# fjall-rs/lsm-tree

Measured on AMD Instinct MI355X. Metric: device-resident data-block decode+encode GiB/s, 1 M × 4 KiB blocks, higher is better.
Workload: dtype u8; 1 GPU; BASELINE configs[1]/[2]: encode + decode round trip of 1 M x 4 KiB data blocks, device-resident; blocks_per_gpu=1048576, items_per_gpu=54525952, block_bytes_per_gpu=3953267212, restart_interval=16, key_len=16, val_len=64, parallelism=shard1 (independent block batches, no collective)

## Files before the change

### lsm-tree_amd/csrc/encode.hip

```cpp
#include <hip/hip_runtime.h>

#include <math.h>

#include <algorithm>
#include <cstddef>
#include <type_traits>

#include "block_format.hpp"
#include "decode.hpp"
#include "encode.hpp"
#include "scan.hpp"
#include "fill.hpp"

namespace lsmgpu {

constexpr uint32_t kPlanHuge = 1, kPlanBad = 2, kPlanMedium = 4, kPlanBig = 8;
constexpr uint32_t kPlanHugeGpu = 16;
constexpr uint32_t kImgMedium = 20 * 1024;
constexpr uint32_t kImgBig = 96 * 1024;
constexpr uint32_t kListBigWaves = 8;
constexpr uint32_t kE3HashChunk = 4096;
constexpr uint64_t kListedOne = 1ULL << 40, kOffMask = kListedOne - 1;

struct alignas(16) BlockPlan {
// ... 285 lines not shown
__device__ __forceinline__ ItemMeta load_item(const EncodeParams& P, uint64_t i, bool& bad) {
  ItemMeta m;
  m.ko = koff<kOW>(P, i);
  const uint64_t kl = koff<kOW>(P, i + 1) - m.ko;
  if (kl > 0xFFFF) bad = true;
  m.klen = (uint32_t)min(kl, (uint64_t)0xFFFF);
  m.seq = gload(P.it.seqno, i);
  m.sh = 0;
  m.e = 0;
  if (is_index(P)) {
    m.vo = gload(P.it.handle_off, i);
    m.vl = gload(P.it.handle_size, i);
    m.vt = 0;
  } else {
    m.vo = voff<kOW>(P, i);
    const uint64_t vl = voff<kOW>(P, i + 1) - m.vo;
    m.vt = gload(P.it.vtype, i);
    if (!valid_vtype(m.vt)) bad = true;
    if (!is_tombstone(m.vt) && vl > 0xFFFFFFFFULL) bad = true;
    m.vl = (uint32_t)vl;
  }
  return m;
}

template <int kOW = 0>
__device__ __forceinline__ ItemMeta load_item_lcp(const EncodeParams& P, uint32_t s, uint32_t j, uint32_t ri,
                                                  bool& bad) {
  const uint64_t i = (uint64_t)s + j;
  ItemMeta m = load_item<kOW>(P, i, bad);
  if (!is_index(P) && j % ri != 0) {
    const uint64_t h = (uint64_t)s + (j / ri) * ri;
    const uint64_t hko = koff<kOW>(P, h);
    const uint32_t hkl = (uint32_t)min(koff<kOW>(P, h + 1) - hko, (uint64_t)0xFFFF);
    m.sh = lcp_global(P.it.keys, hko, m.ko, min(hkl, m.klen));
  }
  return m;
}

__device__ __forceinline__ uint32_t head_len(const EncodeParams& P, const ItemMeta& m, bool head) {
  if (is_index(P)) return 1 + leb_len(m.vo) + leb_len(m.vl) + leb_len(m.seq) + leb_len(m.klen);
  return 1 + leb_len(m.seq) + (head ? leb_len(m.klen) : leb_len(m.sh) + leb_len(m.klen - m.sh));
}

__device__ __forceinline__ uint64_t item_record_len(const EncodeParams& P, const ItemMeta& m, bool head) {
  uint64_t rec = head_len(P, m, head) + m.klen - (head ? 0 : m.sh);
  if (!is_index(P) && !is_tombstone(m.vt)) rec += leb_len(m.vl) + (uint64_t)m.vl;
  return rec;
}

template <class D>
__device__ __forceinline__ uint32_t put_leb(D* dst, uint32_t pos, uint64_t v) {
  while (v >= 0x80) {
    dst[pos++] = (uint8_t)(v | 0x80);
    v >>= 7;
  }
  dst[pos++] = (uint8_t)v;
  return pos;
}

struct RecordCopy {
  SpanCopy<2> key;
  SpanCopy<5> val;
  uint32_t dpos;
  __device__ __forceinline__ void issue(const EncodeParams& P, const ItemMeta& m, bool head, uint32_t dpos_) {
    dpos = dpos_;
    const uint32_t kfrom = head ? 0 : m.sh;
    const uint32_t kpos = dpos_ + head_len(P, m, head);
    key.load(P.it.keys + m.ko + kfrom, m.klen - kfrom, kpos);
    const bool has_val = !is_index(P) && !is_tombstone(m.vt);
    const uint32_t vpos = kpos + m.klen - kfrom + leb_len(m.vl);
    val.load(P.it.vals + (has_val ? m.vo : 0), has_val ? m.vl : 0, vpos);
  }
  template <class D>
  __device__ __forceinline__ void store(const EncodeParams& P, const ItemMeta& m, bool head, D* dst) const {
    uint32_t pos = dpos;
    if (is_index(P)) {
      dst[pos++] = 0;
      pos = put_leb(dst, pos, m.vo);
      pos = put_leb(dst, pos, m.vl);
      pos = put_leb(dst, pos, m.seq);
      put_leb(dst, pos, m.klen);
    } else {
      dst[pos++] = (uint8_t)m.vt;
      pos = put_leb(dst, pos, m.seq);
      if (head) {
        put_leb(dst, pos, m.klen);
      } else {
        pos = put_leb(dst, pos, m.sh);
        put_leb(dst, pos, m.klen - m.sh);
      }
      if (!is_tombstone(m.vt)) put_leb(dst, key.d + key.n, m.vl);
    }
    key.store(dst);
    val.store(dst);
  }
};

template <class D>
__device__ __forceinline__ void store_le(D* dst, uint32_t pos, uint64_t v, uint32_t n) {
  for (uint32_t k = 0; k < n; ++k) dst[pos + k] = (uint8_t)(v >> (8 * k));
}

__device__ __forceinline__ uint32_t key_bucket(const EncodeParams& P, uint64_t ko, uint32_t klen, uint32_t buckets) {
  const uint64_t ka = (uint64_t)(uintptr_t)P.it.keys + ko;
  const uint8_t* kb = reinterpret_cast<const uint8_t*>(ka & ~15ULL);
  const uint32_t kq = (uint32_t)(ka & 15);
  const uint64_t h = xxh3_64_any(klen, BaseReader8{kb, kq}, BaseReader64{kb, kq});
  return (uint32_t)(h % buckets);
}

__device__ __forceinline__ uint32_t bucket_byte(uint32_t lo, uint32_t hi) {
  return lo == 0xFFFFFFFFu ? kHashFree : (lo == hi ? lo : kHashConflict);
}

__device__ __forceinline__ void write_trailer_bytes(uint8_t* dst, uint32_t tp, uint32_t ri, uint32_t step,
                                                    uint32_t bin_len, uint32_t bin_off, uint32_t hash_w,
                                                    uint32_t hash_off, uint32_t items) {
  const int lane = threadIdx.x & 63;
  if (lane >= (int)kTrailerLen) return;
  uint32_t v;
  const int k = lane;
  if (k == 0) v = ri;
  else if (k == 1) v = step;
  else if (k < 6) v = bin_len >> (8 * (k - 2));
  else if (k < 10) v = bin_off >> (8 * (k - 6));
  else if (k < 14) v = hash_w >> (8 * (k - 10));
  else if (k < 18) v = hash_off >> (8 * (k - 14));
  else if (k == 18) v = 1;
  else if (k < 27) v = 0;
  else v = items >> (8 * (k - 27));
  dst[tp + k] = (uint8_t)v;
}

__device__ __forceinline__ void write_header_bytes(uint8_t* dst, uint32_t hp, uint32_t type, uint64_t ck_lo,
                                                   uint64_t ck_hi, uint32_t plen) {
  uint64_t w0 = 0x034D534CULL | ((uint64_t)type << 32) | (ck_lo << 40);
  uint64_t w1 = (ck_lo >> 24) | (ck_hi << 40);
  uint64_t w2 = (ck_hi >> 24) | ((uint64_t)plen << 40);
  uint64_t w3 = ((uint64_t)plen >> 24) | ((uint64_t)plen << 8);
  auto r64 = [&](uint32_t o) -> uint64_t {
    const uint32_t q = o >> 3, sft = (o & 7) * 8;
    const uint64_t a = q == 0 ? w0 : q == 1 ? w1 : q == 2 ? w2 : w3;
    const uint64_t b = q == 0 ? w1 : q == 1 ? w2 : q == 2 ? w3 : 0;
    return sft ? (a >> sft) | (b << (64 - sft)) : a;
  };
  auto r8 = [&](uint32_t o) -> uint32_t { return (uint32_t)(r64(o) & 0xFF); };
  uint64_t hlo, hhi;
  xxh3_128_short(29, r8, r64, hlo, hhi);
  const int lane = threadIdx.x & 63;
  if (lane < 29) dst[hp + lane] = (uint8_t)r8(lane);
  else if (lane < 33) dst[hp + lane] = (uint8_t)((uint32_t)hlo >> (8 * (lane - 29)));
}

__device__ __forceinline__ void write_header_quad(uint8_t* dst, uint32_t hp, uint32_t type, uint64_t ck_lo,
                                                  uint64_t ck_hi, uint32_t plen, int q) {
  const uint64_t w0 = 0x034D534CULL | ((uint64_t)type << 32) | (ck_lo << 40);
  const uint64_t w1 = (ck_lo >> 24) | (ck_hi << 40);
  const uint64_t w2 = (ck_hi >> 24) | ((uint64_t)plen << 40);
  const uint64_t w3 = ((uint64_t)plen >> 24) | ((uint64_t)plen << 8);
  auto r64 = [&](uint32_t o) -> uint64_t {
    const uint32_t qq = o >> 3, sft = (o & 7) * 8;
    const uint64_t a = qq == 0 ? w0 : qq == 1 ? w1 : qq == 2 ? w2 : w3;
    const uint64_t b = qq == 0 ? w1 : qq == 1 ? w2 : qq == 2 ? w3 : 0;
    return sft ? (a >> sft) | (b << (64 - sft)) : a;
  };
  auto r8 = [&](uint32_t o) -> uint32_t { return (uint32_t)(r64(o) & 0xFF); };
  uint64_t hlo, hhi;
  xxh3_128_short(29, r8, r64, hlo, hhi);
  const uint64_t w = q == 0 ? w0 : q == 1 ? w1 : q == 2 ? w2 : (w3 & 0xFFFFFFFFFFULL) | (hlo << 40);
  const uint32_t at = hp + 8 * q;
#pragma unroll
  for (uint32_t i = 0; i < 8; ++i) dst[at + i] = (uint8_t)(w >> (8 * i));
  if (q == 0) dst[hp + 32] = (uint8_t)(hlo >> 24);
}

__device__ __forceinline__ void wave_lds_sync() {
  __builtin_amdgcn_fence(__ATOMIC_RELEASE, "wavefront", "local");
  __builtin_amdgcn_wave_barrier();
  __builtin_amdgcn_fence(__ATOMIC_ACQUIRE, "wavefront", "local");
}

__device__ __forceinline__ void finish_block_lds(const EncodeParams& P, uint32_t b, const BlockPlan& pl, uint32_t n,
                                                 uint32_t ri, uint8_t* img, const uint32_t* hlo, const uint32_t* hhi,
                                                 uint32_t pad, uint32_t total, uint8_t* gdst) {
  const int lane = threadIdx.x & 63;
  const uint32_t step = pl.step_flags & 0xFF;
  const uint32_t plen = total - kHdrLen, p0 = pad + kHdrLen, bin_off = pl.recs + 1;
  if (lane == 0) img[p0 + pl.recs] = kTrailerMarker;
  const uint32_t hash_off = pl.hash_w ? bin_off + pl.bin_len * step : 0;
  for (uint32_t k = lane; k < pl.hash_w; k += kWave) img[p0 + hash_off + k] = (uint8_t)bucket_byte(hlo[k], hhi[k]);
  write_trailer_bytes(img, p0 + plen - kTrailerLen, ri, step, pl.bin_len, bin_off, pl.hash_w, hash_off, n);
  wave_lds_sync();
  if (!(kDiagBuild && (P.diag & 2))) {
    uint64_t ck_lo, ck_hi;
    xxh3_128_wave(img, p0, plen, &kLongSecret, ck_lo, ck_hi);
    write_header_bytes(img, pad, P.type, ck_lo, ck_hi, plen);
  }
  wave_lds_sync();
  const uint32_t chunks = (kDiagBuild && (P.diag & 4)) ? 0 : (pad + total + 15) >> 4;
  for (uint32_t c = lane; c < chunks; c += kWave) {
    const uint32_t lo = c * 16, hi = lo + 16;
    if (lo >= pad && hi <= pad + total) {
      copy_store16(reinterpret_cast<u32x4*>(gdst) + c, reinterpret_cast<const u32x4*>(img)[c]);
    } else {
      for (uint32_t k = max(lo, pad); k < min(hi, pad + total); ++k) gdst[k] = img[k];
    }
  }
  if (lane == 0) P.status[b] = ST_OK;
}

template <int kOW>
__device__ __forceinline__ void write_block_lds(const EncodeParams& P, uint32_t b, uint8_t* smem) {
  const int lane = threadIdx.x & 63;
  const uint32_t s = P.starts[b], e = P.starts[b + 1];
  const uint64_t dst_off = P.block_off[b], dst_end = P.block_off[b + 1];
  const BlockPlan pl = P.plans[b];
  const uint32_t step = pl.step_flags & 0xFF;
  if (dst_end > P.out_cap) {
    if (lane == 0) P.status[b] = ST_OVERFLOW;
    return;
  }
  const uint32_t n = e - s;
  const uint32_t ri = is_index(P) ? 1 : P.ri;
  const uint32_t total = (uint32_t)(dst_end - dst_off);
  const uint64_t dabs = (uint64_t)(uintptr_t)P.out + dst_off;
  const uint32_t pad = (uint32_t)(dabs & 15);
  uint8_t* img = smem;
  uint32_t* hlo = reinterpret_cast<uint32_t*>(smem + ((pad + total + 15) & ~15u) + 32);
  uint32_t* hhi = hlo + ((pl.hash_w + 3) & ~3u);
  for (uint32_t k = lane; k < pl.hash_w; k += kWave) {
    hlo[k] = 0xFFFFFFFFu;
    hhi[k] = 0;
  }
  wave_lds_sync();
  const uint32_t p0 = pad + kHdrLen;
  const uint32_t bin_off = pl.recs + 1;
  uint32_t carry = 0;
  for (uint32_t c = 0; c < n; c += kWave) {
    const uint32_t j = c + lane;
    const bool head = j % ri == 0;
    ItemMeta m;
    RecordCopy rc;
    uint32_t rec = 0;
    if (j < n) {
      bool bad = false;
      m = load_item_lcp<kOW>(P, s, j, ri, bad);
      rec = (uint32_t)item_record_len(P, m, head);
    }
    const uint32_t incl = wave_incl_scan_u32(rec);
    const uint32_t roff = carry + incl - rec;
    if (j < n) {
      rc.issue(P, m, head, p0 + roff);
      rc.store(P, m, head, img);
      if (head) store_le(img, p0 + bin_off + (j / ri) * step, roff, step);
      if (pl.hash_w) {
        const uint32_t bk = key_bucket(P, m.ko, m.klen, pl.hash_w);
        atomicMin(&hlo[bk], j / ri);
        atomicMax(&hhi[bk], j / ri);
      }
    }
    carry += wave_bcast_u32(incl, 63);
  }
  wave_lds_sync();
  finish_block_lds(P, b, pl, n, ri, img, hlo, hhi, pad, total, reinterpret_cast<uint8_t*>(dabs & ~15ULL));
}

template <uint32_t kLW, int kOW>
__device__ __forceinline__ void write_block_lds_mw(const EncodeParams& P, uint32_t b, uint8_t* smem, uint32_t* psum,
                                                   uint64_t* contrib) {
  constexpr uint32_t kT = kLW * kWave;
  const uint32_t tid = threadIdx.x, lane = tid & (kWave - 1);
  const uint32_t wave = __builtin_amdgcn_readfirstlane(tid / kWave);
  const uint32_t s = P.starts[b], e = P.starts[b + 1];
  const uint64_t dst_off = P.block_off[b], dst_end = P.block_off[b + 1];
  const BlockPlan pl = P.plans[b];
  const uint32_t step = pl.step_flags & 0xFF;
  if (dst_end > P.out_cap) {
    if (tid == 0) P.status[b] = ST_OVERFLOW;
    return;
  }
  const uint32_t n = e - s;
  const uint32_t ri = is_index(P) ? 1 : P.ri;
  const uint32_t total = (uint32_t)(dst_end - dst_off);
  const uint64_t dabs = (uint64_t)(uintptr_t)P.out + dst_off;
  const uint32_t pad = (uint32_t)(dabs & 15);
  uint8_t* img = smem;
  uint32_t* hlo = reinterpret_cast<uint32_t*>(smem + ((pad + total + 15) & ~15u) + 32);
  uint32_t* hhi = hlo + ((pl.hash_w + 3) & ~3u);
  for (uint32_t k = tid; k < pl.hash_w; k += kT) {
    hlo[k] = 0xFFFFFFFFu;
    hhi[k] = 0;
  }
  __syncthreads();
  const uint32_t p0 = pad + kHdrLen;
  const uint32_t bin_off = pl.recs + 1;
  uint32_t carry = 0;
  for (uint32_t c = 0; c < n; c += kT) {
    const uint32_t j = c + tid;
    const bool head = j % ri == 0;
    ItemMeta m;
    RecordCopy rc;
    uint32_t rec = 0;
    if (j < n) {
      bool bad = false;
      m = load_item_lcp<kOW>(P, s, j, ri, bad);
      rec = (uint32_t)item_record_len(P, m, head);
    }
// ... 421 lines not shown
          else
            hb = kNeedHash, P.hb_fix[0] = 1;
        }
        P.hbucket[(uint64_t)base + t0 + q] = (uint16_t)hb;
      }
    }
    wave_lds_sync();
    uint32_t nq[kPW];
    uint64_t hq[kPW];
#pragma unroll
    for (uint32_t q = 0; q < kPW; ++q) {
      nq[q] = 0;
      hq[q] = 0;
      wa[q] = wb[q];
      if (ok[q] && jjq[q] % ri != 0) {
        const uint32_t h = base + t0 + q - jjq[q] % ri;
        const bool in = h >= base;
        const uint64_t hko = in ? (uint64_t)wkos[h - base] : hk_ko;
        const uint32_t hkl = in ? wkls[h - base] : hk_kl;
        nq[q] = min(hkl, m[q].klen);
        hq[q] = hko;
        wa[q] = in ? wkwin[h - base] : hk_win;
      }
    }
#pragma unroll
    for (uint32_t q = 0; q < kPW; ++q) {
      if (!nq[q]) continue;
      const uint64_t x0 = wa[q].lo ^ wb[q].lo, x1 = wa[q].hi ^ wb[q].hi;
      const uint32_t n = nq[q];
      uint32_t sh;
      if (x0) sh = min(n, (uint32_t)(__builtin_ctzll(x0) >> 3));
      else if (x1) sh = min(n, 8 + (uint32_t)(__builtin_ctzll(x1) >> 3));
      else sh = n <= 16 ? n : lcp_tail(P.it.keys, hq[q], m[q].ko, n);
      m[q].sh = sh;
    }
    uint64_t rec[kPW], tsum = 0;
#pragma unroll
    for (uint32_t q = 0; q < kPW; ++q) {
      rec[q] = ok[q] ? item_record_len(P, m[q], jjq[q] % ri == 0) : 0;
      tsum += rec[q];
    }
    const uint64_t incl = wave_incl_scan_u64(tsum);
    uint64_t ex = carry + incl - tsum;
    uint64_t exq[kPW];
#pragma unroll
    for (uint32_t q = 0; q < kPW; ++q) {
      exq[q] = ex;
      if (ok[q]) {
        const uint32_t jb = jq[q], jj = jjq[q], ridx = jj / ri;
        const uint32_t n = bst[jb + 1] - bst[jb];
        if (jj == 0) bfirst[jb] = ex;
        if (jj + 1 == n) bend[jb] = ex + rec[q];
        if (jj == ridx * ri && ridx == (n - 1) / ri) lhead[jb] = ex;
      }
      ex += rec[q];
    }
    wave_lds_sync();
#pragma unroll
    for (uint32_t q = 0; q < kPW; ++q) {
      if (ok[q]) {
        const uint32_t jj = jjq[q], ridx = jj / ri;
        const bool head = jj == ridx * ri;
        const uint64_t roff = exq[q] - bfirst[jq[q]];
        const uint32_t x = head ? ridx : m[q].sh;
        P.erec[(uint64_t)base + t0 + q] =
            bst[jq[q] + 1] - bst[jq[q]] > kGItems
                ? (uint32_t)min(roff, (uint64_t)0xFFFFFFFFu)
                : (uint32_t)min(roff, (uint64_t)0x7FFF) | (head ? kErecHead : 0u) | (min(x, 0xFFFFu) << 16);
      }
    }
    carry += wave_bcast_u64(incl, kWave - 1);
    {
      const uint32_t last = min(ie, base + kPWStep) - 1, ll = (last - base) / kPW, lq = (last - base) % kPW;
      uint32_t jsel = jjq[0];
#pragma unroll
      for (uint32_t q = 1; q < kPW; ++q) jsel = lq == q ? jjq[q] : jsel;
      const uint32_t jjl = __builtin_amdgcn_readlane((int)jsel, (int)ll);
      const uint32_t h = last - jjl % ri;
      if (h >= base) {
        hk_ko = wkos[h - base];
        hk_kl = wkls[h - base];
        hk_win = wkwin[h - base];
      }
    }
    wave_lds_sync();
  }
  __syncthreads();
  if (tid >= nb) return;
  const uint32_t b = b0 + tid, s = bst[tid], e = bst[tid + 1];
  bool bad = !mono || e <= s || badf[tid] || start_past_items(P, b + 1);
  const uint32_t n = bad ? 0 : e - s;
  const uint64_t recs = bad ? 0 : bend[tid] - bfirst[tid], last_head = bad ? 0 : lhead[tid] - bfirst[tid];
  const uint32_t bin_len = n ? (n + ri - 1) / ri : 0;
  const uint32_t step = last_head <= 0xFFFF ? 2 : 4;
  const uint32_t buckets = bucket_count(n, P.ratio);
  const uint32_t hash_w = (buckets > 0 && bin_len <= kHashMaxPointers) ? buckets : 0;
  const uint64_t total = kHdrLen + recs + 1 + (uint64_t)bin_len * step + hash_w + kTrailerLen;
  if (recs > 0xFFFFFFF0ULL || total > 0xFFFFFF00ULL) bad = true;
  const uint64_t ks = koff<kOW>(P, s), ke = koff<kOW>(P, e);
  const uint64_t vs = voff<kOW>(P, s), ve = voff<kOW>(P, e);
  uint32_t flags = 0;
  if (bad) {
    flags = kPlanBad;
    P.status[b] = ST_BAD_ARG;
  } else if (!group_fits(n, ke - ks, ve - vs, total, hash_w)) {
    const uint64_t need = e2_need(total, hash_w);
    flags = need <= kImgMedium ? kPlanMedium : need <= kImgBig ? kPlanBig : kPlanHuge;
  }
  const BlockPlan pl{(uint32_t)recs, bin_len, hash_w, step | (flags << 8)};
  const uint64_t size = (bad ? 0 : total) | ((flags & (kPlanMedium | kPlanBig | kPlanHuge)) ? kListedOne : 0);
  P.plans[b] = pl;
  if (kFused) {
    fplan[tid] = pl;
    fsize[tid] = size;
    if (size & ~kOffMask) P.status[b] = ST_INCOMPLETE;
  } else {
    P.sizes[b] = size;
  }
  P.kspan[b] = ks;
  P.vspan[b] = vs;
  if (b + 1 == P.n_blocks) {
    P.kspan[b + 1] = ke;
    P.vspan[b + 1] = ve;
  }
}

template <bool kBkt, int kOW>
__global__ __launch_bounds__(256) __attribute__((amdgpu_waves_per_eu(4))) void encode_plan_wave_kernel(EncodeParams P) {
  __shared__ PlanWaveLds S;
  const uint32_t b0 = blockIdx.x * P.plan_bpw;
  plan_wave_run<kBkt, kOW, false>(P, b0, min(P.plan_bpw, P.n_blocks - b0), S, nullptr, nullptr);
}

struct GBlk {
  uint32_t it0, n;
  uint32_t img, plen;
  uint32_t recs, bin_len;
  uint32_t step, hash_w;
  uint32_t hash_base, u0;
  uint32_t nbk, spare;
};
static_assert(sizeof(GBlk) == 48, "GBlk");

#ifdef LSM_NO_WAVE_BLOCKS
constexpr bool kWaveBlocks = false;
#else
constexpr bool kWaveBlocks = true;
#endif
constexpr uint32_t kWKeys = 1024, kWVals = 4096, kWImg = 4496;
constexpr uint32_t kWItems = kWave;
constexpr uint32_t kWUnits = 5;
static_assert((kWImg - 1) / 1024 <= 4 && (kWImg - 1) / 1024 + 1 <= kWUnits,
              "full KiB units and the tail unit of a payload");
constexpr uint32_t kDiagNoWaveBlocks = 0x20;
struct WaveSlot {
  uint8_t keys[kWKeys + kGSlack];
  uint8_t vals[kWVals + kGSlack];
  uint8_t img[kWImg + kGSlack];
  uint64_t contrib[kWUnits * 8];
};
static_assert(offsetof(WaveSlot, vals) % 16 == 0 && offsetof(WaveSlot, img) % 16 == 0 && sizeof(WaveSlot) % 16 == 0,
              "stage DMA and 16-B copy-out alignment");
constexpr uint32_t kGroupBody = kGKeys + kGVals + kGImg + 3 * kGSlack + kGUnion + 2 * kGBlocks * (uint32_t)sizeof(GBlk);
constexpr uint32_t kWaveSlots = kGWaves * (uint32_t)sizeof(WaveSlot);
constexpr uint32_t kWavePad = kWaveSlots > kGroupBody ? kWaveSlots - kGroupBody : 16;

struct GroupLds {
  uint8_t keys[kGKeys + kGSlack];
  uint8_t vals[kGVals + kGSlack];
  uint8_t img[kGImg + kGSlack];
  uint32_t uni[kGUnion / 4];
  GBlk blk[2][kGBlocks];
  uint8_t wave_pad[kWavePad];
  LongSecret secret;
};
static_assert(offsetof(GroupLds, uni) - offsetof(GroupLds, vals) >= sizeof(PlanWaveLds), "plan LDS over the stage");
static_assert(offsetof(GroupLds, vals) % 16 == 0, "plan LDS alignment");
static_assert(kGRunFused * (sizeof(BlockPlan) + 8) + 16 <= kGUnion, "fused plan outputs in uni");
static_assert(offsetof(GroupLds, wave_pad) == kGroupBody, "GroupLds layout");
static_assert(kGWaves * sizeof(WaveSlot) <= offsetof(GroupLds, secret), "the wave slots lie over the group loop's LDS");
static_assert(sizeof(GroupLds) <= 40960, "four workgroups per CU");

__device__ __host__ __forceinline__ bool wave_fits(uint64_t n, uint64_t kspan, uint64_t vspan, uint64_t total) {
  return n >= 1 && n <= kWItems && kspan + 15 <= kWKeys && vspan + 15 <= kWVals && total + 15 <= kWImg;
}


__device__ __forceinline__ void lds_copy(uint8_t* dst, uint32_t d, const uint8_t* src, uint32_t s, uint32_t n,
                                         uint32_t rot, uint32_t done = 0) {
  if (!n) return;
  const uint32_t h = min(n, (4u - (d & 3u)) & 3u);
  uint32_t hb[3];
#pragma unroll
  for (uint32_t k = 0; k < 3; ++k)
    if (k < h) hb[k] = src[s + k];
#pragma unroll
  for (uint32_t k = 0; k < 3; ++k)
    if (k < h) dst[d + k] = (uint8_t)hb[k];
  if (n == h) return;
  const uint32_t d1 = d + h + 4 * done, e = d + n, body = ((e & ~3u) - d1) >> 2;
  const uint32_t sp = s + h + 4 * done, sh = sp & 3u;
  const uint32_t* s32 = reinterpret_cast<const uint32_t*>(src + (sp & ~3u));
  uint32_t* d32 = reinterpret_cast<uint32_t*>(dst + d1);
  uint32_t q = ((rot & 31u) * body) >> 5;
  constexpr uint32_t U = 4;
  const uint32_t w0 = body ? s32[0] : 0;
  uint32_t carry = body ? s32[q] : 0;
  for (uint32_t j0 = 0; j0 < body; j0 += U) {
    uint32_t hi[U], at[U];
#pragma unroll
    for (uint32_t t = 0; t < U; ++t) {
      uint32_t p = q + t;
      p = p >= body ? p - body : p;
      at[t] = p;
      if (j0 + t < body) hi[t] = s32[p + 1];
    }
#pragma unroll
    for (uint32_t t = 0; t < U; ++t) {
      if (j0 + t < body) {
        const uint32_t lo = t == 0 ? carry : (at[t] == 0 ? w0 : hi[t - 1]);
        d32[at[t]] = alignbyte(hi[t], lo, sh);
      }
    }
    q += U;
    q = q >= body ? q - body : q;
    carry = q == 0 ? w0 : hi[U - 1];
  }
  const uint32_t t0 = d1 + 4 * body;
  uint32_t tb[3];
#pragma unroll
  for (uint32_t k = 0; k < 3; ++k)
    if (t0 + k < e) tb[k] = src[s + (t0 + k - d)];
#pragma unroll
  for (uint32_t k = 0; k < 3; ++k)
    if (t0 + k < e) dst[t0 + k] = (uint8_t)tb[k];
}

#ifdef LSM_NO_UNIFORM_COPY
constexpr bool kUniformCopy = false;
#else
constexpr bool kUniformCopy = true;
#endif
constexpr uint32_t kUniformMin = 4;
__device__ __forceinline__ uint32_t lds_copy_uniform(uint8_t* dst, uint32_t d, const uint8_t* src, uint32_t s,
                                                     uint32_t n, bool has, uint32_t rot) {
  if (!kUniformCopy) return 0;
  const uint32_t h = min(n, (4u - (d & 3u)) & 3u);
  const uint32_t body = n > h ? (((d + n) & ~3u) - (d + h)) >> 2 : 0u;
  const uint32_t B = wave_min_u32(has ? body : 0xFFFFFFFFu);
  if (B < kUniformMin || B == 0xFFFFFFFFu) return 0;
  if (has) {
    const uint8_t* sb = src + ((s + h) & ~3u);
    uint8_t* db = dst + d + h;
    const uint32_t sh = (s + h) & 3u, B4 = 4 * B;
    auto ld = [&](uint32_t x) { return *reinterpret_cast<const uint32_t*>(sb + x); };
    auto st = [&](uint32_t x, uint32_t v) { *reinterpret_cast<uint32_t*>(db + x) = v; };
    constexpr uint32_t U = kUniformMin;
    uint32_t x = (((rot & 31u) * B) >> 5) * 4;
    const uint32_t w0 = ld(0);
    uint32_t carry = ld(x);
    for (uint32_t j = 0; j < B; j += U) {
      uint32_t at[U], hi[U];
#pragma unroll
      for (uint32_t t = 0; t < U; ++t) {
        const uint32_t y = x + 4 * t;
        at[t] = t == 0 ? x : min(y, y - B4);
        hi[t] = ld(at[t] + 4);
      }
#pragma unroll
      for (uint32_t t = 0; t < U; ++t) {
        const uint32_t lo = at[t] == 0 ? w0 : (t == 0 ? carry : hi[t - 1]);
        st(at[t], alignbyte(hi[t], lo, sh));
      }
      carry = hi[U - 1];
      x += 4 * U;
      x = min(x, x - B4);
    }
    if (body > B) {
      st(B4, alignbyte(ld(B4 + 4), ld(B4), sh));
      return B + 1;
    }
  }
  return B;
}

__device__ __forceinline__ uint32_t lds_put_leb(uint8_t* dst, uint32_t pos, uint64_t v) {
  while (v >= 0x80) {
    dst[pos++] = (uint8_t)(v | 0x80);
    v >>= 7;
  }
  dst[pos++] = (uint8_t)v;
  return pos;
}

template <bool kIndex>
__device__ __forceinline__ uint32_t put_record_header(uint8_t* img, uint32_t pos, const uint8_t* keys, uint32_t kst,
                                                      const ItemMeta& m, bool head, uint32_t from, uint32_t rot) {
  if (kIndex) {
    img[pos++] = 0;
    pos = lds_put_leb(img, pos, m.vo);
    pos = lds_put_leb(img, pos, m.vl);
    pos = lds_put_leb(img, pos, m.seq);
    pos = lds_put_leb(img, pos, m.klen);
    lds_copy(img, pos, keys, kst, m.klen, rot);
  } else {
    img[pos++] = (uint8_t)m.vt;
// ... 398 lines not shown
    }
    const uint32_t cs = in_run ? clamped_start(P, rb) : 0;
    r_ks = in_run ? koff<kOW>(P, cs) : 0;
    r_vs = in_run ? voff<kOW>(P, cs) : 0;
    __syncthreads();
  } else {
    r_off = in_run ? P.block_off[rb] : 0;
    r_ks = in_run ? P.kspan[rb] : 0;
    r_vs = in_run ? P.vspan[rb] : 0;
    r_plan = (in_run && rb < b_end) ? P.plans[rb] : BlockPlan{0, 0, 0, 0};
  }
  const uint32_t r_hash = r_plan.hash_w;
  const uint32_t r_hpre = wave_incl_scan_u32(r_hash) - r_hash;
  uint32_t r_upre;
  {
    const uint64_t nx = wave_shfl_u64(r_off, min(lane + 1, 63));
    const uint32_t plen = (rb < b_end) ? (uint32_t)(nx - r_off) - kHdrLen : 0;
    const uint32_t units = plen > 240 ? (plen - 1) / 1024 + 1 : 0;
    r_upre = wave_incl_scan_u32(units) - units;
  }
  auto lane_u32 = [&](uint32_t v, uint32_t l) { return (uint32_t)__shfl((int)v, (int)min(l, 63u)); };
  auto lane_u64 = [&](uint64_t v, uint32_t l) { return wave_shfl_u64(v, (int)min(l, 63u)); };
  auto rl32 = [&](uint32_t v, uint32_t l) { return (uint32_t)__builtin_amdgcn_readlane((int)v, (int)min(l, 63u)); };
  auto rl64 = [&](uint64_t v, uint32_t l) {
    const int q = (int)min(l, 63u);
    return (uint64_t)(uint32_t)__builtin_amdgcn_readlane((int)(uint32_t)v, q) |
           ((uint64_t)(uint32_t)__builtin_amdgcn_readlane((int)(uint32_t)(v >> 32), q) << 32);
  };
  struct Grp {
    uint32_t b, k;
  };
  auto form = [&](uint32_t b) -> Grp {
    const uint32_t r0 = b - b_begin, rj = r0 + lane;
    const uint32_t s0 = rl32(r_start, r0), s1 = lane_u32(r_start, rj + 1);
    const uint64_t o0 = rl64(r_off, r0), o1 = lane_u64(r_off, rj + 1);
    const uint64_t k0 = rl64(r_ks, r0), k1 = lane_u64(r_ks, rj + 1);
    const uint64_t v0 = rl64(r_vs, r0), v1 = lane_u64(r_vs, rj + 1);
    const uint32_t flags = lane_u32(r_plan.step_flags, rj) >> 8;
    const uint32_t hsum = lane_u32(r_hpre, rj + 1) - rl32(r_hpre, r0);
    const bool ok = b + lane < b_end && lane < (int)kGBlocks && flags == 0 && o1 <= P.out_cap &&
                    group_fits(s1 - s0, k1 - (k0 & ~15ULL), v1 - (v0 & ~15ULL), o1 - (o0 & ~15ULL), hsum);
    return Grp{b, (uint32_t)__builtin_ctzll(~__ballot(ok))};
  };
  const uint64_t gmask = __ballot(rb < b_end && (r_plan.step_flags >> 8) == 0);
  auto next_group = [&](uint32_t b) -> Grp {
    for (;;) {
      if (b >= b_end) return Grp{b, 0};
      const Grp g = form(b);
      if (g.k) return g;
      const uint64_t rest = gmask >> (b - b_begin);
      if (rest & 1) {
        if (lane == 0) P.status[b] = ST_OVERFLOW;
        ++b;
      } else {
        b = rest ? b + (uint32_t)__builtin_ctzll(rest) : b_end;
      }
    }
  };
  auto issue_dma = [&](const Grp& g) {
    const uint32_t r0 = g.b - b_begin;
    const uint64_t ka = rl64(r_ks, r0) & ~15ULL, kb = rl64(r_ks, r0 + g.k);
    const uint64_t va = rl64(r_vs, r0) & ~15ULL, vb = rl64(r_vs, r0 + g.k);
    const uint32_t kc = (uint32_t)((kb - ka + 15) >> 4), vc = index ? 0 : (uint32_t)((vb - va + 15) >> 4);
    stage_to_lds(P.it.keys + ka, L.keys, kc, wave, kGWaves, lane);
    stage_to_lds(P.it.vals + va, L.vals, vc, wave, kGWaves, lane);
  };
  uint32_t* hlo = L.uni;
  uint32_t* hhi = hlo + kGHash;
  uint64_t* contrib = reinterpret_cast<uint64_t*>(L.uni);

  auto tpi_shift = [&](uint32_t n) -> uint32_t { return n <= kGThreads / 4 ? 2u : n <= kGThreads / 2 ? 1u : 0u; };
  auto load_items = [&](const Grp& g, RawItemT<kOW, kIndex>& r) {
    const uint32_t r0 = g.b - b_begin;
    const uint32_t i0 = rl32(r_start, r0), n = rl32(r_start, r0 + g.k) - i0;
    const uint64_t i = (uint64_t)i0 + min(tid >> tpi_shift(n), n - 1);
    r = load_raw<kIndex, kOW>(P, i);
    r.e = P.erec[i];
    if (kPlanBkt) r.hb = P.hbucket[i];
  };
  auto cook = [&](const RawItemT<kOW, kIndex>& r) {
    bool bad = false;
    return cook_item<kIndex>(r, bad);
  };

  auto build_table = [&](const Grp& g, GBlk* tb) {
    const uint32_t gr0 = g.b - b_begin, gk = g.k;
    const uint32_t gi0 = rl32(r_start, gr0);
    const uint64_t gob = rl64(r_off, gr0);
    const uint32_t gpad = (uint32_t)(((uint64_t)(uintptr_t)P.out + gob) & 15);
    const uint32_t rj = gr0 + lane;
    const uint32_t st = lane_u32(r_start, rj), st1 = lane_u32(r_start, rj + 1);
    const uint64_t of = lane_u64(r_off, rj), of1 = lane_u64(r_off, rj + 1);
    const uint32_t recs = lane_u32(r_plan.recs, rj), bin_len = lane_u32(r_plan.bin_len, rj);
    const uint32_t sf = lane_u32(r_plan.step_flags, rj), hw = lane_u32(r_plan.hash_w, rj);
    const uint32_t hb = lane_u32(r_hpre, rj) - rl32(r_hpre, gr0);
    const bool in = (uint32_t)lane < gk;
    const uint32_t plen = in ? (uint32_t)(of1 - of) - kHdrLen : 0;
    const uint32_t nbk = plen > 240 ? (plen - 1) / 1024 : 0;
    const uint32_t units = plen > 240 ? nbk + 1 : 0;
    const uint32_t u0 = wave_incl_scan_u32(units) - units;
    if (in) {
      GBlk B;
      B.it0 = st - gi0;
      B.n = st1 - st;
      B.img = (uint32_t)(of - gob) + gpad;
      B.plen = plen;
      B.recs = recs;
      B.bin_len = bin_len;
      B.step = sf & 0xFF;
      B.hash_w = hw;
      B.hash_base = hb;
      B.u0 = u0;
      B.nbk = nbk;
      B.spare = 0;
      tb[lane] = B;
    }
  };

  constexpr bool kWaveLoop = kWaveBlocks && !kIndex && !kHash && !kPlanBkt && !kFused;
  if constexpr (kWaveLoop) {
    bool wave_run;
    {
      const uint32_t s1 = lane_u32(r_start, lane + 1);
      const uint64_t o1 = lane_u64(r_off, lane + 1), k1 = lane_u64(r_ks, lane + 1), v1 = lane_u64(r_vs, lane + 1);
      const bool fit = (r_plan.step_flags >> 8) == 0 && o1 <= P.out_cap &&
                       wave_fits(s1 - r_start, k1 - (r_ks & ~15ULL), v1 - (r_vs & ~15ULL), o1 - (r_off & ~15ULL));
      wave_run = __ballot(rb < b_end && !fit) == 0 && !(kDiagBuild && (P.diag & (kDiagNoWaveBlocks | 0x9F)));
    }
    if (wave_run) {
      WaveSlot& W = reinterpret_cast<WaveSlot*>(&L)[wave];
      auto wave_lds_wait = [&]() { asm volatile("s_waitcnt lgkmcnt(0)" ::: "memory"); };
      auto wave_dma = [&](uint32_t r) {
        const uint64_t ka = rl64(r_ks, r) & ~15ULL, kb = rl64(r_ks, r + 1);
        const uint64_t va = rl64(r_vs, r) & ~15ULL, vb = rl64(r_vs, r + 1);
        const uint32_t kc = (uint32_t)((kb - ka + 15) >> 4), vc = (uint32_t)((vb - va + 15) >> 4);
        stage_to_lds(P.it.keys + ka, W.keys, kc, 0, 1, lane);
        stage_to_lds(P.it.vals + va, W.vals, vc, 0, 1, lane);
      };
      auto wave_items = [&](uint32_t r, RawItemT<kOW, kIndex>& x) {
        const uint32_t i0 = rl32(r_start, r), n = rl32(r_start, r + 1) - i0;
        const uint64_t i = (uint64_t)i0 + min((uint32_t)lane, n - 1);
        x = load_raw<kIndex, kOW>(P, i);
        x.e = P.erec[i];
      };
      group_barrier_lds();
      uint32_t r = wave;
      const uint32_t nr = b_end - b_begin;
      RawItemT<kOW, kIndex> raw{};
      if (r < nr) {
        wave_dma(r);
        wave_items(r, raw);
      }
      vm_wait<0>();
      while (r < nr) {
        const uint32_t i0 = rl32(r_start, r), n = rl32(r_start, r + 1) - i0;
        const uint64_t kbase = rl64(r_ks, r) & ~15ULL, vbase = rl64(r_vs, r) & ~15ULL;
        const uint64_t obase = rl64(r_off, r);
        const uint32_t total = (uint32_t)(rl64(r_off, r + 1) - obase), plen = total - kHdrLen;
        const uint32_t recs = rl32(r_plan.recs, r), bin_len = rl32(r_plan.bin_len, r);
        const uint32_t step = rl32(r_plan.step_flags, r) & 0xFF;
        const uint64_t dabs = (uint64_t)(uintptr_t)P.out + obase;
        const uint32_t pad = (uint32_t)(dabs & 15), p0 = pad + kHdrLen;
        const uint32_t rn = r + kGWaves;
        const bool more = rn < nr;
        ItemMeta m = cook(raw);
        if (more) wave_items(rn, raw);
        {
          const bool live = (uint32_t)lane < n;
          const bool head = (m.e & kErecHead) != 0;
          m.sh = head ? 0u : m.e >> 16;
          const uint32_t roff = m.e & 0x7FFFu, from = head ? 0 : m.sh;
          const uint32_t kst = (uint32_t)(m.ko - kbase), vsrc = (uint32_t)(m.vo - vbase);
          const bool has_val = live && !is_tombstone(m.vt);
          uint32_t vpos = 0;
          if (live) vpos = put_record_header<false>(W.img, p0 + roff, W.keys, kst, m, head, from, lane);
          const uint32_t done = lds_copy_uniform(W.img, vpos, W.vals, vsrc, m.vl, has_val && m.vl != 0, lane);
          if (live) {
            if (has_val) lds_copy(W.img, vpos, W.vals, vsrc, m.vl, lane, done);
            if (head) put_bin_entry(W.img, p0 + recs + 1 + (m.e >> 16) * step, step, roff);
          }
        }
        if (lane == 0) W.img[p0 + recs] = kTrailerMarker;
        write_trailer_bytes(W.img, p0 + plen - kTrailerLen, ri, step, bin_len, recs + 1, 0, 0, n);
        wave_lds_wait();
        if (more) wave_dma(rn);
        uint64_t lo = 0, hi = 0;
        const int q = lane & 3;
        if (plen > 240) {
          const uint32_t nbk = (plen - 1) / 1024;
          {
            const uint32_t row = (uint32_t)lane >> 4, rr = lane & 15;
            for (uint32_t u = row; u <= nbk; u += 4) {
              uint64_t c0, c1;
              xxh3_row_unit(W.img, p0, plen, nbk, u, rr, &L.secret, c0, c1);
              if (rr < 4) {
                W.contrib[8 * u + 2 * q] = c0;
                W.contrib[8 * u + 2 * q + 1] = c1;
              }
            }
          }
          wave_lds_wait();
          uint64_t a0, a1;
          xxh3_acc_init(q, a0, a1);
          const uint64_t scr0 = L.secret.acc[16 + 2 * q], scr1 = L.secret.acc[16 + 2 * q + 1];
          static_assert((kWImg - 1) / 1024 <= 4 && 4 <= kWUnits, "nbk <= 4");
          const uint64_t* cb = W.contrib + 2 * q;
          const uint64_t t0 = cb[8 * nbk], t1 = cb[8 * nbk + 1];
          xxh3_quad_chain_batch<4>(cb, 0, nbk, scr0, scr1, a0, a1);
          a0 += t0;
          a1 += t1;
          xxh3_merge_part(&L.secret, q, a0, a1, lo, hi);
        }
        lo = quad_sum64(lo);
        hi = quad_sum64(hi);
        if (lane < 4) {
          if (plen > 240) {
            xxh3_finish128(plen, lo, hi, lo, hi);
          } else {
            xxh3_128_short(plen, BaseReader8{W.img, p0}, BaseReader64{W.img, p0}, lo, hi);
          }
          write_header_quad(W.img, pad, P.type, lo, hi, plen, q);
          if (lane == 0) P.status[b_begin + r] = ST_OK;
        }
        wave_lds_wait();
        vm_wait<0>();
        {
          const uint32_t end = pad + total, c0 = (pad + 15) >> 4, c1 = end >> 4;
          const u32x4* const csrc = reinterpret_cast<const u32x4*>(W.img);
          u32x4* const cdst = reinterpret_cast<u32x4*>(dabs & ~15ULL);
          for (uint32_t c = c0 + (uint32_t)lane; c < c1; c += kWave)
            *(__attribute__((address_space(1))) u32x4*)(cdst + c) = csrc[c];
          auto* gb = (__attribute__((address_space(1))) uint8_t*)cdst;
          const uint32_t x = (uint32_t)lane;
          if (x >= pad && x < min(16 * c0, end)) gb[x] = W.img[x];
          if (c1 >= c0 && 16 * c1 + x < end) gb[16 * c1 + x] = W.img[16 * c1 + x];
        }
        wave_lds_wait();
        r = rn;
      }
      return;
    }
  }

#ifdef LSM_DIAG
  uint64_t t_last = __builtin_amdgcn_s_memtime();
  uint32_t ph_acc[12] = {};
  uint32_t ph_n = 0;
#endif
  Grp G = run_ok ? next_group(b_begin) : Grp{b_end, 0};
  RawItemT<kOW, kIndex> raw{};
  if (G.k) {
    issue_dma(G);
    load_items(G, raw);
    if (wave == 0) build_table(G, L.blk[0]);
  }
  vm_lgkm_wait0();
  ENC_PHASE(11);
  uint32_t iter = 0;
  while (G.k) {
    ENC_PHASE(0);
    const uint32_t r0 = G.b - b_begin, k = G.k;
    const uint32_t i0 = rl32(r_start, r0), n_items = rl32(r_start, r0 + k) - i0;
    const uint64_t kbase = rl64(r_ks, r0) & ~15ULL, vbase = rl64(r_vs, r0) & ~15ULL;
    const uint64_t obase = rl64(r_off, r0);
    const uint64_t dabs = (uint64_t)(uintptr_t)P.out + obase;
    const uint32_t pad = (uint32_t)(dabs & 15);
    const uint32_t tsh = tpi_shift(n_items), part = tid & ((1u << tsh) - 1), item = tid >> tsh;
    const bool live = item < n_items;
    const Grp Gn = next_group(G.b + k);
    ItemMeta m = cook(raw);
    if (Gn.k) load_items(Gn, raw);
    ENC_PHASE(9);
    GBlk* const TB = L.blk[iter & 1];
    const uint32_t hsum = rl32(r_hpre, r0 + k) - rl32(r_hpre, r0);
    for (uint32_t h = tid; h < hsum; h += kGThreads) {
      hlo[h] = 0xFFFFFFFFu;
      hhi[h] = 0;
    }
    group_barrier_lds();
    ENC_PHASE(1);
    uint32_t j = 0;
    for (uint32_t jb = 1; jb < k; ++jb) j += (rl32(r_start, r0 + jb) - i0 <= item) ? 1u : 0u;
    const bool head = (m.e & kErecHead) != 0;
    m.sh = head ? 0u : m.e >> 16;
    const bool writes = live && !(kDiagBuild && (P.diag & 9));
    const uint32_t roff = m.e & 0x7FFFu;
    const uint32_t from = head ? 0 : m.sh;
    const uint32_t kst = (uint32_t)(m.ko - kbase);
    const bool has_val = writes && !index && !is_tombstone(m.vt);
    const uint32_t vsrc = (uint32_t)(m.vo - vbase);
    auto put_header = [&]() -> uint32_t {
      return put_record_header<index>(L.img, TB[j].img + kHdrLen + roff, L.keys, kst, m, head, from, lane);
    };
    auto put_index_and_vote = [&]() {
      const GBlk& B = TB[j];
      if (head) put_bin_entry(L.img, B.img + kHdrLen + B.recs + 1 + (m.e >> 16) * B.step, B.step, roff);
      if (kHash && B.hash_w) {
        const uint32_t ridx = (item - B.it0) / ri;
        const uint32_t hb =
            kPlanBkt ? m.hb
                     : (uint32_t)(xxh3_64_any(m.klen, BaseReader8{L.keys, kst}, BaseReader64{L.keys, kst}) % B.hash_w);
        const uint32_t bk = B.hash_base + hb;
        atomicMin(&hlo[bk], ridx);
        atomicMax(&hhi[bk], ridx);
      }
    };
    constexpr bool uniform = !index;
    if (tsh == 0) {
      uint32_t vpos = 0;
      if (writes) vpos = put_header();
      const uint32_t done =
          uniform ? lds_copy_uniform(L.img, vpos, L.vals, vsrc, m.vl, has_val && m.vl != 0, lane) : 0u;
      if (writes) {
        if (has_val) lds_copy(L.img, vpos, L.vals, vsrc, m.vl, lane, done);
        put_index_and_vote();
      }
    } else {
      const uint32_t va = (part * m.vl) >> tsh, vb = ((part + 1) * m.vl) >> tsh;
      uint32_t vpos = 0;
      if (writes) {
        if (part == 0)
          vpos = put_header();
        else if (has_val)
          vpos = TB[j].img + kHdrLen + roff + 1 + leb_len(m.seq) + (head ? 0u : leb_len(m.sh)) + leb_len(m.klen - from) +
                 (m.klen - from) + leb_len(m.vl);
      }
      const uint32_t done =
          uniform ? lds_copy_uniform(L.img, vpos + va, L.vals, vsrc + va, vb - va, has_val && vb != va, lane) : 0u;
      if (writes) {
        if (has_val) lds_copy(L.img, vpos + va, L.vals, vsrc + va, vb - va, lane, done);
        if (part == 0) put_index_and_vote();
      }
    }
    auto tails = [&]() {
      for (uint32_t jb = wave; jb < (kDiagBuild && (P.diag & 8) ? 0 : k); jb += kGWaves) {
        const GBlk& B = TB[jb];
        const uint32_t p0 = B.img + kHdrLen, bin_off = B.recs + 1;
        if (lane == 0) L.img[p0 + B.recs] = kTrailerMarker;
        const uint32_t hash_off = B.hash_w ? bin_off + B.bin_len * B.step : 0;
        if (kHash)
          for (uint32_t q = lane; q < B.hash_w; q += kWave)
            L.img[p0 + hash_off + q] = (uint8_t)bucket_byte(hlo[B.hash_base + q], hhi[B.hash_base + q]);
        write_trailer_bytes(L.img, p0 + B.plen - kTrailerLen, ri, B.step, B.bin_len, bin_off, B.hash_w, hash_off,
                            B.n);
      }
    };
    if (!kHash) tails();
    group_barrier_lds();
    ENC_PHASE(3);
    if (Gn.k && !(kDiagBuild && (P.diag & 16))) issue_dma(Gn);
    ENC_PHASE(10);
    if (kHash) {
      tails();
      group_barrier_lds();
    }
    ENC_PHASE(4);
    {
      const uint32_t row = wave * 4 + (lane >> 4), r = lane & 15, q = r & 3;
      const uint32_t ubase = rl32(r_upre, r0);
      const uint32_t units = (kDiagBuild && (P.diag & 10)) ? 0 : rl32(r_upre, r0 + k) - ubase;
      for (uint32_t u = row; u < units; u += 4 * kGWaves) {
        uint32_t jb = 0;
        for (uint32_t x = 1; x < k; ++x) jb += (rl32(r_upre, r0 + x) - ubase <= u) ? 1u : 0u;
        const GBlk& B = TB[jb];
        uint64_t c0, c1;
        xxh3_row_unit(L.img, B.img + kHdrLen, B.plen, B.nbk, u - B.u0, r, &L.secret, c0, c1);
        if (r < 4) {
          contrib[8 * u + 2 * q] = c0;
          contrib[8 * u + 2 * q + 1] = c1;
        }
      }
    }
    group_barrier_lds();
    ENC_PHASE(5);
    const uint32_t cw = iter & (kGWaves - 1);
    const uint32_t total = (uint32_t)(rl64(r_off, r0 + k) - obase);
    const uint32_t end = (kDiagBuild && (P.diag & 4)) ? pad : pad + total;
    const uint32_t c0 = (pad + 15) >> 4, c1 = end >> 4;
    const u32x4* const csrc = reinterpret_cast<const u32x4*>(L.img);
    u32x4* const cdst = reinterpret_cast<u32x4*>(dabs & ~15ULL);
    const uint32_t hpc = (wave == cw && (uint32_t)lane < 3 * k) ? (TB[lane / 3].img >> 4) + lane % 3 : ~0u;
    if (wave == cw) {
      if (!(kDiagBuild && (P.diag & 10))) {
        const uint32_t jb = (uint32_t)lane >> 2;
        const int q = lane & 3;
        const bool in = jb < k;
        const GBlk& B = TB[in ? jb : 0];
        const uint32_t p0 = B.img + kHdrLen, plen = B.plen;
        uint64_t lo = 0, hi = 0;
        if (in && plen > 240) {
// ... 826 lines not shown
```

Baseline: 973.9 GiB/s.

## Defer per-block header checksum finalize and batch four blocks across lane quads

In the wave-per-block encode path, the final xxh3 chain/merge/finish and header write used to run on only four lanes per block, followed by an extra LDS wait. This change keeps each block's per-unit contributions in registers and hashes short payloads on a designated lane quad. Every four blocks it flushes them together, one lane quad per block, and writes the 32-byte header straight to global memory. The aim is to use the wave's lanes better for the serial finalize and drop one LDS sync per block. In exchange it adds register pressure, a flush-time LDS staging step, and small unaligned global header stores.

```diff
diff --git a/lsm-tree_amd/csrc/encode.hip b/lsm-tree_amd/csrc/encode.hip
--- a/lsm-tree_amd/csrc/encode.hip
+++ b/lsm-tree_amd/csrc/encode.hip
@@ -461,7 +461,8 @@
   else if (lane < 33) dst[hp + lane] = (uint8_t)((uint32_t)hlo >> (8 * (lane - 29)));
 }
 
-__device__ __forceinline__ void write_header_quad(uint8_t* dst, uint32_t hp, uint32_t type, uint64_t ck_lo,
+template <class BytePtr>
+__device__ __forceinline__ void write_header_quad(BytePtr dst, uint32_t hp, uint32_t type, uint64_t ck_lo,
                                                   uint64_t ck_hi, uint32_t plen, int q) {
   const uint64_t w0 = 0x034D534CULL | ((uint64_t)type << 32) | (ck_lo << 40);
   const uint64_t w1 = (ck_lo >> 24) | (ck_hi << 40);
@@ -1189,6 +1190,9 @@
 constexpr uint32_t kWUnits = 5;
 static_assert((kWImg - 1) / 1024 <= 4 && (kWImg - 1) / 1024 + 1 <= kWUnits,
               "full KiB units and the tail unit of a payload");
+constexpr uint32_t kWDefer = 4;
+static_assert(kWDefer >= 1 && kWDefer <= kWave / 4, "one lane quad per deferred block");
+static_assert(kWDefer * kWUnits * 8 * 8 <= kWImg, "the kept contributions fit the free image at the flush");
 constexpr uint32_t kDiagNoWaveBlocks = 0x20;
 struct WaveSlot {
   uint8_t keys[kWKeys + kGSlack];
@@ -1893,6 +1897,50 @@
         wave_items(r, raw);
       }
       vm_wait<0>();
+      uint64_t d0 = 0, d1 = 0;
+      uint64_t kc[kWDefer] = {};
+      uint32_t dn = 0, dr = wave;
+      auto flush_headers = [&]() {
+        const uint32_t rj = dr + kGWaves * ((uint32_t)lane >> 2);
+        const int q = lane & 3;
+        const bool in = ((uint32_t)lane >> 2) < dn;
+        const uint64_t ob = lane_u64(r_off, rj);
+        const uint32_t plen = (uint32_t)(lane_u64(r_off, rj + 1) - ob) - kHdrLen;
+        const bool lng = in && plen > 240;
+        uint64_t lo = 0, hi = 0;
+        constexpr uint32_t kCW = kWUnits * 8;
+        uint64_t* const side = reinterpret_cast<uint64_t*>(W.img);
+        if ((uint32_t)lane < kCW) {
+#pragma unroll
+          for (uint32_t s = 0; s < kWDefer; ++s) side[kCW * s + (uint32_t)lane] = kc[s];
+        }
+        wave_lds_wait();
+        if (lng) {
+          const uint32_t nbk = (plen - 1) / 1024;
+          uint64_t a0, a1;
+          xxh3_acc_init(q, a0, a1);
+          const uint64_t scr0 = L.secret.acc[16 + 2 * q], scr1 = L.secret.acc[16 + 2 * q + 1];
+          static_assert((kWImg - 1) / 1024 <= 4 && 4 <= kWUnits, "nbk <= 4: one batch is the whole chain");
+          const uint64_t* cb = side + kCW * ((uint32_t)lane >> 2) + 2 * q;
+          const uint64_t t0 = cb[8 * nbk], t1 = cb[8 * nbk + 1];
+          xxh3_quad_chain_batch<4>(cb, 0, nbk, scr0, scr1, a0, a1);
+          d0 = a0 + t0;
+          d1 = a1 + t1;
+        }
+        if (lng) xxh3_merge_part(&L.secret, q, d0, d1, lo, hi);
+        lo = quad_sum64(lo);
+        hi = quad_sum64(hi);
+        if (in) {
+          if (lng) {
+            xxh3_finish128(plen, lo, hi, lo, hi);
+          } else {
+            lo = d0;
+            hi = d1;
+          }
+          write_header_quad((__attribute__((address_space(1))) uint8_t*)(P.out + ob), 0, P.type, lo, hi, plen, q);
+          if (q == 0) P.status[b_begin + rj] = ST_OK;
+        }
+      };
       while (r < nr) {
         const uint32_t i0 = rl32(r_start, r), n = rl32(r_start, r + 1) - i0;
         const uint64_t kbase = rl64(r_ks, r) & ~15ULL, vbase = rl64(r_vs, r) & ~15ULL;
@@ -1925,8 +1973,6 @@
         write_trailer_bytes(W.img, p0 + plen - kTrailerLen, ri, step, bin_len, recs + 1, 0, 0, n);
         wave_lds_wait();
         if (more) wave_dma(rn);
-        uint64_t lo = 0, hi = 0;
-        const int q = lane & 3;
         if (plen > 240) {
           const uint32_t nbk = (plen - 1) / 1024;
           {
@@ -1935,48 +1981,39 @@
               uint64_t c0, c1;
               xxh3_row_unit(W.img, p0, plen, nbk, u, rr, &L.secret, c0, c1);
               if (rr < 4) {
-                W.contrib[8 * u + 2 * q] = c0;
-                W.contrib[8 * u + 2 * q + 1] = c1;
+                W.contrib[8 * u + 2 * rr] = c0;
+                W.contrib[8 * u + 2 * rr + 1] = c1;
               }
             }
           }
           wave_lds_wait();
-          uint64_t a0, a1;
-          xxh3_acc_init(q, a0, a1);
-          const uint64_t scr0 = L.secret.acc[16 + 2 * q], scr1 = L.secret.acc[16 + 2 * q + 1];
-          static_assert((kWImg - 1) / 1024 <= 4 && 4 <= kWUnits, "nbk <= 4");
-          const uint64_t* cb = W.contrib + 2 * q;
-          const uint64_t t0 = cb[8 * nbk], t1 = cb[8 * nbk + 1];
-          xxh3_quad_chain_batch<4>(cb, 0, nbk, scr0, scr1, a0, a1);
-          a0 += t0;
-          a1 += t1;
-          xxh3_merge_part(&L.secret, q, a0, a1, lo, hi);
+          {
+            const uint64_t cv = W.contrib[min((uint32_t)lane, kWUnits * 8 - 1)];
+#pragma unroll
+            for (uint32_t s = 0; s < kWDefer; ++s) kc[s] = dn == s ? cv : kc[s];
+          }
+        } else if (((uint32_t)lane >> 2) == dn) {
+          xxh3_128_short(plen, BaseReader8{W.img, p0}, BaseReader64{W.img, p0}, d0, d1);
         }
-        lo = quad_sum64(lo);
-        hi = quad_sum64(hi);
-        if (lane < 4) {
-          if (plen > 240) {
-            xxh3_finish128(plen, lo, hi, lo, hi);
-          } else {
-            xxh3_128_short(plen, BaseReader8{W.img, p0}, BaseReader64{W.img, p0}, lo, hi);
-          }
-          write_header_quad(W.img, pad, P.type, lo, hi, plen, q);
-          if (lane == 0) P.status[b_begin + r] = ST_OK;
-        }
-        wave_lds_wait();
+        ++dn;
         vm_wait<0>();
         {
-          const uint32_t end = pad + total, c0 = (pad + 15) >> 4, c1 = end >> 4;
+          const uint32_t end = pad + total, ch = (p0 + 15) >> 4, c1 = end >> 4;
           const u32x4* const csrc = reinterpret_cast<const u32x4*>(W.img);
           u32x4* const cdst = reinterpret_cast<u32x4*>(dabs & ~15ULL);
-          for (uint32_t c = c0 + (uint32_t)lane; c < c1; c += kWave)
+          for (uint32_t c = ch + (uint32_t)lane; c < c1; c += kWave)
             *(__attribute__((address_space(1))) u32x4*)(cdst + c) = csrc[c];
           auto* gb = (__attribute__((address_space(1))) uint8_t*)cdst;
           const uint32_t x = (uint32_t)lane;
-          if (x >= pad && x < min(16 * c0, end)) gb[x] = W.img[x];
-          if (c1 >= c0 && 16 * c1 + x < end) gb[16 * c1 + x] = W.img[16 * c1 + x];
+          if (p0 + x < min(16 * ch, end)) gb[p0 + x] = W.img[p0 + x];
+          if (c1 >= ch && 16 * c1 + x < end) gb[16 * c1 + x] = W.img[16 * c1 + x];
         }
         wave_lds_wait();
+        if (dn == kWDefer || !more) {
+          flush_headers();
+          dn = 0;
+          dr = rn;
+        }
         r = rn;
       }
       return;
```

Result: faster. 1008 GiB/s (median of 6 runs) (+3.5%).
